# microsoft/ConfigNet

Hardware: AMD Instinct MI355X
Metric: train-step images/sec at 256x256 (G+D fwd+bwd) (higher is better)
Workload: dtype f32; 1 GPU; ConfigNet second-stage iteration (D + synth-D + latent-D + G + EMA), 256x256, batch 16 per GPU, fp32, Keras-Adam; global_batch=16, resolution=256, latent_dim=145, parallelism=dp1, losses_finite=True

## Files before the change

### confignet_amd/_lib.py

```python
import ctypes
import os

_HERE = os.path.dirname(os.path.abspath(__file__))
LIB_PATH = os.environ.get("CN_LIB") or os.path.join(_HERE, "libconfignet_hip.so")


class CnSumJob(ctypes.Structure):
    _fields_ = [("src", ctypes.c_void_p), ("dst", ctypes.c_void_p), ("count", ctypes.c_longlong), ("parts", ctypes.c_int),
                ("accumulate", ctypes.c_int)]


class CnDepthJob(ctypes.Structure):
    _fields_ = [("a", ctypes.c_void_p), ("b", ctypes.c_void_p), ("c", ctypes.c_void_p), ("m", ctypes.c_int), ("n", ctypes.c_int),
                ("k", ctypes.c_int), ("lda", ctypes.c_int), ("ldb", ctypes.c_int), ("ldc", ctypes.c_int)]


class CnRowsJob(ctypes.Structure):
    _fields_ = [("a", ctypes.c_void_p), ("b", ctypes.c_void_p), ("c", ctypes.c_void_p), ("bias", ctypes.c_void_p), ("mask", ctypes.c_void_p)] + \
               [(n_, ctypes.c_int) for n_ in ("m", "n", "k", "lda", "ldb", "ldc", "tb", "act", "accumulate")] + [("slope", ctypes.c_float)]


class CnGanJob(ctypes.Structure):
    _fields_ = [("s", ctypes.c_void_p), ("out", ctypes.c_void_p), ("gout", ctypes.c_void_p), ("n", ctypes.c_int), ("label", ctypes.c_float)]

# ... 40 lines not shown
    "cn_conv_wgrad_thin_partials": [],
    "cn_conv_wgrad_thin": [_G, _p, _p, _p, _p, _i, _p],
    "cn_conv_wgrad": [_G, _p, _p, _p, _i, _p],
    "cn_conv_wgrad_workspace_bytes": [_G],
    "cn_conv_wgrad_ws": [_G, _p, _p, _p, _i, _p, _z, _p],
    "cn_conv_wgrad_ws_slabs": [_G, _p, _p, _p, _i, _p, _z, ctypes.POINTER(_i), _p],
    "cn_conv_wgrad_dt_workspace_bytes": [_G, _i, _i, ctypes.POINTER(_z)],
    "cn_conv_wgrad_dt": [_G, _p, _i, _p, _i, _p, _i, _p, _z, ctypes.POINTER(_i), _p],
    "cn_conv_wgrad_plan": [_G, _i, _i, _i, ctypes.c_uint, _i, ctypes.POINTER(ctypes.c_longlong)],
    "cn_sum_parts_grouped": [_p, _i, _p],
    "cn_gemm_depth_grouped": [_p, _i, _p],
    "cn_gan_loss_grouped": [_p, _i, _i, _p],
    "cn_gemm_rows_grouped": [_p, _i, _p],
    "cn_conv_tune": [_i, _i, ctypes.c_long],
    "cn_conv_fwd_plan": [_G, _i, _i, _i, _i, _i, _i, _i, ctypes.POINTER(ctypes.c_int * 8)],
    "cn_conv_loop_select": [_i, _i, _i, _i],
    "cn_conv_fwd_dt": [_p, _p, _i, _p, _p, _p, _i, _i, _f, _p],
    "cn_conv_dgrad_dt": [_p, _p, _i, _p, _p, _i, _p],
    "cn_conv_wgrad_c3_partials": [],
    "cn_conv_wgrad_c3": [_p, _p, _p, _i, _p, _p, _i, _p],
    "cn_conv_wino_filter": [_p, _p, _i, _i, _i, _p],
    "cn_conv_fwd_wino": [_i, _i, _i, _i, _i, _p, _p, _p, _p, _i, _f, _p],
    "cn_conv_fwd_wino4": [_i, _i, _i, _i, _i, _p, _p, _p, _p, _i, _f, _p],
    "cn_conv_wino4_filter": [_p, _p, _i, _i, _i, _p],
    "cn_sumpool2": [_p, _p, _i, _i, _i, _i, _i, _i, _i, _p],
    "cn_gemm": [_i, _i, _i, _i, _i, _p, _i, _p, _i, _p, _i, _p, _i, _f, _p],
    "cn_gemm_plan": [_i] * 10 + [ctypes.POINTER(ctypes.c_int * 9)],
    "cn_nc_reduce4": [_p, _p, _i, _i, _i, _f, _i, _i, _p],
    "cn_nc_reduce": [_p, _p, _p, _p, _i, _i, _i, _i, _f, _i, _p],
    "cn_nc_reduce_plan": [_i, _i, _i, _i, _i, _i, ctypes.POINTER(ctypes.c_int * 8)],
    "cn_nc_lin2": [_p, _p, _p, _p, _p, _p, _p, _p, _i, _i, _i, _i, _i, _f, _i, _p],
    "cn_nc_rows_plan": [ctypes.c_longlong, _i, _i, ctypes.POINTER(ctypes.c_int * 2)],
    "cn_norm_coef_fwd": [_i, _p, _p, _p, _p, _p, _p, _p, _p, _i, _i, _i, _f, _p, _i, _p],
    "cn_norm_coef_bwd": [_i, _p, _p, _p, _p, _p, _p, _p, _p, _p, _p, _i, _i, _i, _f, _p],
    "cn_dual_tail_coef_fwd": [_p] * 13 + [_i, _i, _i, _f, _i, _i, _p],
    "cn_dual_tail_coef_bwd": [_p] * 13 + [ctypes.POINTER(ctypes.c_void_p), _i, _i, _i, _f, _i, _i, _p],
    "cn_dual_tail_gx": [_p] * 12 + [_i, _i, _i, _f, _i, _i, _p],
    "cn_dual_tail_gx_tx": [_p] * 18 + [_i, _i, _i, _f, _i, _i, _i, _p],
    "cn_norm_apply": [_i, _i] + [_p] * 13 + [_i, _i, _i, _f, _i, _f, _i, _p],
    "cn_nc_reduce_hxt": [_p, _p, _p, _p, _i, _i, _i, _f, _i, _i, _i, _p],
    "cn_zero": [_p, ctypes.c_size_t, _p],
    "cn_set_deterministic": [_i],
    "cn_get_deterministic": [],
    "cn_det_release_stream": [_p],
    "cn_gemm_acc": [_i, _i, _i, _i, _i, _p, _i, _p, _i, _p, _i, _p],
    "cn_sum_rows_into": [_p, _p, _i, _i, _i, _p],
# ... 61 lines not shown
```

### confignet_amd/csrc/common.h

```cpp
#pragma once
#include <hip/hip_runtime.h>
#include <stdint.h>
#include <stdio.h>
#include "../../include/confignet_hip.h"

void cn_set_error(const char* fmt, ...);

#define CN_CHECK_ARG(cond, ...)            \
    do {                                   \
        if (!(cond)) {                     \
            cn_set_error(__VA_ARGS__);     \
            return CN_EINVAL;              \
        }                                  \
    } while (0)

#define CN_HIP(expr)                                                              \
    do {                                                                          \
        hipError_t e__ = (expr);                                                  \
        if (e__ != hipSuccess) {                                                  \
            cn_set_error("%s failed: %s (%s:%d)", #expr, hipGetErrorString(e__), __FILE__, __LINE__); \
            return CN_EHIP;                                                       \
        }                                                                         \
    } while (0)

// ... 60 lines not shown

__device__ __forceinline__ void divmod_pos(int m, int d, int& q, int& r) {
    if ((d & (d - 1)) == 0) {
        q = m >> (__builtin_ctz(d));
        r = m & (d - 1);
    } else {
        q = m / d;
        r = m - q * d;
    }
}

__device__ __forceinline__ float cn_apply_act(float v, int act, float slope) {
    switch (act) {
        case CN_ACT_LRELU: return v > 0.f ? v : v * slope;
        case CN_ACT_RELU: return v > 0.f ? v : 0.f;
        case CN_ACT_TANH: return tanhf(v);
        default: break;
    }
    if (act == CN_ACT_RELU6) return fminf(fmaxf(v, 0.f), 6.f);
    if (act == CN_ACT_SIGMOID) return __fdividef(1.f, 1.f + __expf(-v));
    return v;
}

static inline int cn_cdiv(long a, long b) { return (int)((a + b - 1) / b); }

int cn_cu_count();
```

### confignet_amd/csrc/elementwise.hip

```cpp
#include "common.h"
#include "typed.h"
#include <stdlib.h>

namespace {

__device__ __forceinline__ float lrelu(float v, float s) { return v > 0.f ? v : v * s; }

__device__ __forceinline__ float act_deriv(float o, int act, float slope) {
    if (act == CN_ACT_LRELU) return o > 0.f ? 1.f : slope;
    if (act == CN_ACT_RELU) return o > 0.f ? 1.f : 0.f;
    if (act == CN_ACT_TANH) return 1.f - o * o;
    return 1.f;
}


template <int V> struct RowV { float v[V]; };

template <int V, typename T>
__device__ __forceinline__ RowV<V> ld_row(const T* p) {
    RowV<V> r;
    if constexpr (V == 4) {
        const float4 t = ld4<T>(p);
        r.v[0] = t.x; r.v[1] = t.y; r.v[2] = t.z; r.v[3] = t.w;
    } else {
        r.v[0] = ldf<T>(p);
    }
    return r;
}
template <int V, typename T>
__device__ __forceinline__ void st_row(T* p, const RowV<V>& r) {
    if constexpr (V == 4) st4<T>(p, make_float4(r.v[0], r.v[1], r.v[2], r.v[3]));
    else stf<T>(p, r.v[0]);
}

template <int Q, int V, typename Op>
__device__ __forceinline__ void nc_reduce_rows(Op op, float* const (&out)[Q], int S, int C, int rows_per_block, float* __restrict__ parts) {
// ... 616 lines not shown
    }
}

template <typename T>
__global__ void maxpool_fwd_kernel(const T* __restrict__ x, T* __restrict__ y, int n, int h, int w, int c,
                                   int oh, int ow, int k, int s, int pad) {
    const long total = (long)n * oh * ow * c;
    for (long i = (long)blockIdx.x * blockDim.x + threadIdx.x; i < total; i += (long)gridDim.x * blockDim.x) {
        const int ch = (int)(i % c);
        long t = i / c;
        const int ox = (int)(t % ow);
        t /= ow;
        const int oy = (int)(t % oh);
        const int b = (int)(t / oh);
        float best = -INFINITY;
        for (int dy = 0; dy < k; ++dy)
            for (int dx = 0; dx < k; ++dx) {
                const int iy = oy * s - pad + dy, ix = ox * s - pad + dx;
                const bool in = iy >= 0 && iy < h && ix >= 0 && ix < w;
                const float v = in ? ldf<T>(x + (((long)b * h + iy) * w + ix) * c + ch) : 0.f;
                if (in || pad > 0) best = fmaxf(best, v);
            }
        stf<T>(y + i, best);
    }
}

template <int V, typename T>
__global__ void avgpool3_same_kernel(const T* __restrict__ x, T* __restrict__ y, int n, int h, int w, int c) {
    const int CG = c / V;
    const long total = (long)n * h * w * CG;
    for (long i = (long)blockIdx.x * blockDim.x + threadIdx.x; i < total; i += (long)gridDim.x * blockDim.x) {
        const int cg = (int)(i % CG);
        long t = i / CG;
        const int ox = (int)(t % w);
        t /= w;
        const int oy = (int)(t % h);
        const int b = (int)(t / h);
        float acc[V];
#pragma unroll
        for (int e = 0; e < V; ++e) acc[e] = 0.f;
        int cnt = 0;
        for (int dy = -1; dy <= 1; ++dy)
            for (int dx = -1; dx <= 1; ++dx) {
                const int iy = oy + dy, ix = ox + dx;
                if (iy < 0 || iy >= h || ix < 0 || ix >= w) continue;
                const T* p = x + (((long)b * h + iy) * w + ix) * c + (long)cg * V;
// ... 552 lines not shown
    CN_LAUNCH_CHECK();
    return CN_OK;
}
extern "C" int cn_tap_bwd(const void* y, const void* target, const void* g, const float* s, void* out, int n, size_t row, float k,
                          int act, float slope, int dt, void* stream) {
    CN_CHECK_ARG(y && target && s && out && n > 0 && row > 0 && (dt == CN_F32 || dt == CN_BF16), "tap_bwd: bad args");
    const int vec = alv(y, dt) && alv(target, dt) && alv(out, dt) && (!g || alv(g, dt)) && row % 4 == 0;
    int bpr = (int)((row + 256 * 16 - 1) / (256 * 16));
    if (bpr > 512) bpr = 512;
    CN_DISPATCH_DT(dt, hipLaunchKernelGGL((tap_bwd_kernel<T>), dim3(bpr, n), dim3(256), 0, (hipStream_t)stream, (const T*)y, (const T*)target,
                                          (const T*)g, s, (T*)out, row, k, vec, act, slope));
    CN_LAUNCH_CHECK();
    return CN_OK;
}
extern "C" int cn_masked_diff(const float* a, const float* b, const uint8_t* mask, float* out, size_t pixels, int c, void* stream) {
    CN_CHECK_ARG(a && mask && out && c > 0, "masked_diff: bad args");
    if (!pixels) return CN_OK;
    EW_LAUNCH(masked_diff_kernel, pixels, a, b, mask, out, pixels, c)
}
extern "C" int cn_maxpool_fwd(const void* x, void* y, int n, int h, int w, int c, int k, int s, int pad, int dt, void* stream) {
    CN_CHECK_ARG(x && y && n > 0 && h > 0 && w > 0 && c > 0 && k > 0 && s > 0 && pad >= 0 && (dt == CN_F32 || dt == CN_BF16), "maxpool: bad args");
    const int oh = (h + 2 * pad - k) / s + 1, ow = (w + 2 * pad - k) / s + 1;
    const size_t total = (size_t)n * oh * ow * c;
    CN_DISPATCH_DT(dt, hipLaunchKernelGGL((maxpool_fwd_kernel<T>), dim3(ew_blocks(total)), dim3(256), 0, (hipStream_t)stream, (const T*)x, (T*)y, n, h, w, c, oh, ow, k, s, pad));
    CN_LAUNCH_CHECK();
    return CN_OK;
}
extern "C" int cn_avgpool3_same(const void* x, void* y, int n, int h, int w, int c, int dt, void* stream) {
    CN_CHECK_ARG(x && y && n > 0 && h > 0 && w > 0 && c > 0 && (dt == CN_F32 || dt == CN_BF16), "avgpool3_same: bad args");
    const bool v4 = c % 4 == 0 && alv(x, dt) && alv(y, dt);
    const size_t total = (size_t)n * h * w * (v4 ? c / 4 : c);
    CN_DISPATCH_DT(dt, {
        if (v4) hipLaunchKernelGGL((avgpool3_same_kernel<4, T>), dim3(ew_blocks(total)), dim3(256), 0, (hipStream_t)stream, (const T*)x, (T*)y, n, h, w, c);
        else hipLaunchKernelGGL((avgpool3_same_kernel<1, T>), dim3(ew_blocks(total)), dim3(256), 0, (hipStream_t)stream, (const T*)x, (T*)y, n, h, w, c);
    });
    CN_LAUNCH_CHECK();
    return CN_OK;
}
extern "C" int cn_maxpool_bwd(const void* x, const void* gy, void* gx, int n, int h, int w, int c, int k, int s, int pad, int dt, void* stream) {
    CN_CHECK_ARG(x && gy && gx && n > 0 && h > 0 && w > 0 && c > 0 && k > 0 && s > 0 && pad >= 0 && (dt == CN_F32 || dt == CN_BF16), "maxpool_bwd: bad args");
    const int oh = (h + 2 * pad - k) / s + 1, ow = (w + 2 * pad - k) / s + 1;
    const size_t total = (size_t)n * h * w * c;
    if (k == 2 && s == 2 && pad == 0 && h % 2 == 0 && w % 2 == 0 && c % 4 == 0 && alv(x, dt) && alv(gy, dt) && alv(gx, dt)) {
        const long windows4 = (long)n * oh * ow * (c / 4);
        CN_DISPATCH_DT(dt, hipLaunchKernelGGL((maxpool2_bwd_kernel<T>), dim3(ew_blocks((size_t)windows4)), dim3(256), 0, (hipStream_t)stream,
                                              (const T*)x, (const T*)gy, (T*)gx, windows4, oh, ow, c / 4));
// ... 206 lines not shown
```

### confignet_amd/csrc/winograd4.hip

```cpp
#include "common.h"

#include "mma_tile.h"

namespace {

typedef __attribute__((address_space(3))) float lds_float4;
typedef float v2f __attribute__((ext_vector_type(2)));

struct Wino4Geom {
    int n, h, w, cin, cout, bh, bw;
};

__global__ void wino4_filter_kernel(const float* __restrict__ W, float* __restrict__ U, int cin, int cout, int dgrad) {
    const long total = (long)cin * cout;
    for (long e = (long)blockIdx.x * blockDim.x + threadIdx.x; e < total; e += (long)gridDim.x * blockDim.x) {
        const int co = (int)(e % cout), ci = (int)(e / cout);
        float g[3][3];
#pragma unroll
        for (int a = 0; a < 3; ++a)
#pragma unroll
            for (int b = 0; b < 3; ++b)
                g[a][b] = dgrad ? W[((long)((2 - a) * 3 + (2 - b)) * cin + ci) * cout + co] : W[((long)(a * 3 + b) * cin + ci) * cout + co];
        float t[6][3];
#pragma unroll
// ... 17 lines not shown
            u[2] = (-1.f / 6.f) * (t0 - t1 + t2);
            u[3] = (1.f / 24.f) * t0 + (1.f / 12.f) * t1 + (1.f / 6.f) * t2;
            u[4] = (1.f / 24.f) * t0 - (1.f / 12.f) * t1 + (1.f / 6.f) * t2;
            u[5] = t2;
#pragma unroll
            for (int b = 0; b < 6; ++b) U[((long)(a * 6 + b) * kdim + k) * ndim + nn] = u[b];
        }
    }
}

#ifndef W4_ABLATE
#define W4_ABLATE 0
#endif
constexpr int W4_KC = 4;
constexpr int W4_T = 32;
constexpr int W4_C = 64;
constexpr int W4_VP = 40;
constexpr int W4_U = 36 * W4_KC * W4_C;
constexpr int W4_RAW_PIECES = 21;
constexpr int W4_RAW = W4_RAW_PIECES * 256;
constexpr int W4_BUF = 2 * W4_U + 2 * W4_RAW;


__global__ __launch_bounds__(768) void wino4_fwd_kernel(Wino4Geom g, const float* __restrict__ X, const float* __restrict__ U,
                                                        const float* __restrict__ bias, float* __restrict__ Y, int act, float slope) {
    __shared__ __attribute__((aligned(16))) float Vs[2][36][W4_KC][W4_VP];
    extern __shared__ __attribute__((aligned(16))) float BUF[];
    const int tid = threadIdx.x, lane = tid & 63, wave = __builtin_amdgcn_readfirstlane(tid >> 6);
    const int half = lane >> 5, l31 = lane & 31;
    const int wi = wave % 6, cb = wave / 6;

    const int nblk = g.n * g.bh * g.bw, total = nblk * (g.cout / W4_C);
    int wg = blockIdx.x;
    if (total % 8 == 0) wg = (wg & 7) * (total >> 3) + (wg >> 3);
    const int blk = wg % nblk, co0 = (wg / nblk) * W4_C;
    int img, brem, by, bx;
    divmod_pos(blk, g.bh * g.bw, img, brem);
    divmod_pos(brem, g.bw, by, bx);

    const __amdgpu_buffer_rsrc_t xres = __builtin_amdgcn_make_buffer_rsrc(const_cast<float*>(X), 0, g.n * g.h * g.w * g.cin * 4, 0x00020000);
    const __amdgpu_buffer_rsrc_t ures = __builtin_amdgcn_make_buffer_rsrc(const_cast<float*>(U), 0, 36 * g.cin * g.cout * 4, 0x00020000);

    unsigned uoff[3];
#pragma unroll
    for (int j = 0; j < 3; ++j) {
        const int p = wave + 12 * j;
        uoff[j] = (unsigned)((p * g.cin + (lane >> 4)) * g.cout + co0 + (lane & 15) * 4) * 4u;
    }
// ... 149 lines not shown
        float t = 0.f;
#pragma unroll
        for (int j = 0; j < 6; ++j)
#pragma unroll
            for (int r = 0; r < 16; ++r) t += acc[j][r];
        if (t == 12345.f) Y[tid] = t;
        return;
    }
    for (int rb = 0; rb < 2; ++rb) {
        if (cb == rb) {
#pragma unroll
            for (int e = 0; e < 16; ++e) {
                const int tl = 4 * half + (e & 3) + 8 * (e >> 2);
                const float a0 = acc[0][e], a1 = acc[1][e], a2 = acc[2][e], a3 = acc[3][e], a4 = acc[4][e], a5 = acc[5][e];
                const float s12 = a1 + a2, d12 = a1 - a2, s34 = a3 + a4, d34 = a3 - a4;
                float* dst = E + ((wi * 4) * 32 + tl) * 32 + l31;
                dst[0 * 1024] = a0 + s12 + s34;
                dst[1 * 1024] = d12 + 2.f * d34;
                dst[2 * 1024] = s12 + 4.f * s34;
                dst[3 * 1024] = d12 + 8.f * d34 + a5;
            }
        }
        __syncthreads();
        for (int idx = tid; idx < 1024; idx += 768) {
            const int c4 = idx & 7, tl = (idx >> 3) & 31, y = idx >> 8;
            float4 m[6];
#pragma unroll
            for (int i = 0; i < 6; ++i) m[i] = *reinterpret_cast<const float4*>(E + ((i * 4 + y) * 32 + tl) * 32 + 4 * c4);
            const int co = co0 + rb * 32 + 4 * c4;
            const float4 bv = bias ? *reinterpret_cast<const float4*>(bias + co) : make_float4(0.f, 0.f, 0.f, 0.f);
            const int otx = (tl & 3) + 4 * ((tl >> 3) & 1), oty = ((tl >> 2) & 1) + 2 * (tl >> 4);
            const int row0 = by * 16 + 4 * oty, col = bx * 32 + 4 * otx + y;
#define W4_O(f)                                                                                                          \
            const float s12##f = m[1].f + m[2].f, d12##f = m[1].f - m[2].f, s34##f = m[3].f + m[4].f, d34##f = m[3].f - m[4].f; \
            const float o0##f = m[0].f + s12##f + s34##f + bv.f, o1##f = d12##f + 2.f * d34##f + bv.f,                     \
                        o2##f = s12##f + 4.f * s34##f + bv.f, o3##f = d12##f + 8.f * d34##f + m[5].f + bv.f;
            W4_O(x) W4_O(y) W4_O(z) W4_O(w)
#undef W4_O
            float* dst = Y + ((long)(img * g.h + row0) * g.w + col) * g.cout + co;
            const long rs = (long)g.w * g.cout;
            *reinterpret_cast<float4*>(dst) = make_float4(cn_apply_act(o0x, act, slope), cn_apply_act(o0y, act, slope), cn_apply_act(o0z, act, slope), cn_apply_act(o0w, act, slope));
            *reinterpret_cast<float4*>(dst + rs) = make_float4(cn_apply_act(o1x, act, slope), cn_apply_act(o1y, act, slope), cn_apply_act(o1z, act, slope), cn_apply_act(o1w, act, slope));
            *reinterpret_cast<float4*>(dst + 2 * rs) = make_float4(cn_apply_act(o2x, act, slope), cn_apply_act(o2y, act, slope), cn_apply_act(o2z, act, slope), cn_apply_act(o2w, act, slope));
            *reinterpret_cast<float4*>(dst + 3 * rs) = make_float4(cn_apply_act(o3x, act, slope), cn_apply_act(o3y, act, slope), cn_apply_act(o3z, act, slope), cn_apply_act(o3w, act, slope));
        }
        __syncthreads();
    }
}

}

extern "C" int cn_conv_wino4_filter(const float* w, float* u, int cin, int cout, int dgrad, void* stream) {
    CN_CHECK_ARG(w && u && cin > 0 && cout > 0, "wino4_filter: bad args");
    const long total = (long)cin * cout;
    const int blocks = (int)((total + 255) / 256 > 4096 ? 4096 : (total + 255) / 256);
    hipLaunchKernelGGL(wino4_filter_kernel, dim3(blocks), dim3(256), 0, (hipStream_t)stream, w, u, cin, cout, dgrad);
    CN_LAUNCH_CHECK();
    return CN_OK;
}

extern "C" int cn_conv_fwd_wino4(int n, int h, int w, int cin, int cout, const float* x, const float* u, const float* bias,
                                 float* y, int act, float slope, void* stream) {
    CN_CHECK_ARG(x && u && y && n > 0 && h > 0 && w > 0, "conv_fwd_wino4: bad args");
    if (h % 16 || w % 32 || cin % 16 || cout % W4_C) return CN_EUNSUPPORTED;
    CN_CHECK_ARG((double)n * h * w * (cin > cout ? cin : cout) * 4.0 < 2147483647.0 && 144.0 * cin * cout < 2147483647.0,
                 "tensor exceeds 2^31 bytes (buffer descriptors, 32-bit offsets)");
    Wino4Geom g{n, h, w, cin, cout, h / 16, w / 32};
    const long nblk = (long)n * g.bh * g.bw;
    constexpr size_t lds = sizeof(float) * W4_BUF;
    static bool attr_set = false;
    if (!attr_set) {
        CN_HIP(hipFuncSetAttribute(reinterpret_cast<const void*>(wino4_fwd_kernel), hipFuncAttributeMaxDynamicSharedMemorySize, (int)lds));
        attr_set = true;
    }
    hipStream_t s = (hipStream_t)stream;
    cn_prof_begin(s, 2.0 * 36.0 * (double)nblk * W4_T * cin * cout, 4.0 * ((double)n * h * w * (cin + cout) + 36.0 * cin * cout), CN_FAM_WINO);
    hipLaunchKernelGGL(wino4_fwd_kernel, dim3((unsigned)(nblk * (cout / W4_C))), dim3(768), lds, s, g, x, u, bias, y, act, slope);
    cn_prof_end(s);
    CN_LAUNCH_CHECK();
    return CN_OK;
}
```

### confignet_amd/dnn_models/vgg.py

```python
import numpy as np
import torch

from .. import functional as F
from ..nn import Net, he_normal
from ..ops import ACT_RELU, ConvSpec

VGG19_CFG = [64, 64, "P", 128, 128, "P", 256, 256, 256, 256, "P", 512, 512]
VGG16_CFG = [64, 64, "P", 128, 128, "P", 256, 256, 256, "P", 512, 512]
VGG19_TAPS = (0, 1, 5, 9)
VGG16_TAPS = (0, 1, 5, 8)
C3 = ConvSpec((3, 3))


class VGGFeatures(Net):
    def __init__(self, cfg, taps, rng=None):
        super().__init__()
        rng = rng or np.random.default_rng(1234)
        self.cfg, self.taps = cfg, taps
        cin = 3
        for i, item in enumerate(c for c in cfg if c != "P"):
            self.add_weight("conv%d/kernel" % i, he_normal(rng, (3, 3, cin, item)), trainable=False)
            self.add_weight("conv%d/bias" % i, np.zeros(item, np.float32), trainable=False)
            cin = item
        self.finalize()

    def __call__(self, x_pre):
        feats, ci, x = [], 0, x_pre
        for item in self.cfg:
            if item == "P":
                x = F.maxpool(x, 2, 2)
            else:
                x = F.conv(x, self.weights[2 * ci], self.weights[2 * ci + 1], C3, ACT_RELU)
                if ci in self.taps:
                    feats.append(x)
                ci += 1
        return feats


class VGGLossFn(torch.autograd.Function):

    @staticmethod
    def forward(ctx, net, x, sizes, *targets):
        from .. import ops
        x = x.contiguous()
        ys, feats, ci, t = [], [], 0, x
        for item in net.cfg:
            if item == "P":
                t = ops.maxpool_fwd(t, 2, 2, 0)
            else:
                w, b = net.weights[2 * ci], net.weights[2 * ci + 1]
                t = ops.conv_fwd(t, w, b, C3.geom(tuple(t.shape), w.shape[-1]), ACT_RELU)
                ys.append(t)
                if ci in net.taps:
                    feats.append(t)
                ci += 1
        n = x.shape[0]
        groups = [n] if sizes is None else list(sizes)
        terms = []
        for a, b in zip(feats, targets):
            per = a.numel() // n
            n0, row = 0, []
            for sz in groups:
                row.append(ops.sqdiff_sum(a[n0:n0 + sz], b[n0:n0 + sz], 1.0 / (sz * per)))
                n0 += sz
            terms.append(torch.cat(row) if len(row) > 1 else row[0])
        total = torch.stack(terms).sum(0)
        ctx.net, ctx.sizes, ctx.x_shape = net, sizes, tuple(x.shape)
        ctx.save_for_backward(x, *ys, *targets)
        ctx.counts = (len(ys),)
        return total.reshape(()) if sizes is None else total

    @staticmethod
    def backward(ctx, g):
        from .. import ops
        if torch.is_grad_enabled():
            raise RuntimeError("VGGLossFn is first-order only")
        net, sizes = ctx.net, ctx.sizes
        saved = ctx.saved_tensors
        (ny,) = ctx.counts
        x, ys, targets = saved[0], saved[1:1 + ny], saved[1 + ny:]
        n = x.shape[0]
        g = g.reshape(-1).float()
        tap_of = {ci: k for k, ci in enumerate(net.taps)}
        gcur, ci, pooled = None, ny, None
        for item in reversed(net.cfg):
            if item == "P":
                pooled, gcur = gcur, None
                continue
            ci -= 1
            y = ys[ci]
            s_ = k = None
            if ci in tap_of:
                per = y.numel() // n
                if sizes is None:
                    s_, k = g.contiguous(), 2.0 / (n * per)
                else:
                    s_ = torch.cat([g[i:i + 1].expand(sz) * (1.0 / (sz * per)) for i, sz in enumerate(sizes)]).contiguous()
                    k = 2.0
            gu = None
            if pooled is not None:
                gu = ops.maxpool2_bwd_relu(y, pooled, targets[tap_of[ci]] if s_ is not None else None, s_, k if s_ is not None else 0.0)
                if gu is None:
                    gcur = ops.maxpool_bwd(y, pooled, 2, 2, 0)
                pooled = None
            if gu is not None:
                pass
            elif s_ is not None:
                gu = ops.tap_bwd(y, targets[tap_of[ci]], gcur, s_, k, ACT_RELU)
            elif gcur is None:
                continue
            else:
                gu = ops.act_bwd(gcur, y, ACT_RELU)
            w = net.weights[2 * ci]
            in_shape = conv_input_shape(net.cfg, ci, ctx.x_shape)
            gcur = ops.conv_dgrad(gu, w, C3.geom(in_shape, w.shape[-1]))
        return None, gcur, None, *([None] * len(targets))


def conv_input_shape(cfg, ci, x_shape):
    n, h, w, c = x_shape
    k = -1
    for item in cfg:
        if item == "P":
            h, w = h // 2, w // 2
        else:
            k += 1
            if k == ci:
                return (n, h, w, c)
            c = item
    raise IndexError(ci)
```

### confignet_amd/ops.py

```python
import contextlib
import ctypes
import math
import os
import threading

import torch

from ._lib import CN_BF16, CN_EUNSUPPORTED, CN_F32, CN_U8, CnConvGeom, CnDepthJob, CnGanJob, CnRowsJob, CnSumJob, check, lib

ACT_NONE, ACT_LRELU, ACT_RELU, ACT_TANH, ACT_RELU6, ACT_SIGMOID = 0, 1, 2, 3, 4, 5

ACT_DTYPE = torch.float32


def set_activation_dtype(dtype):
    global ACT_DTYPE
    if isinstance(dtype, str):
        dtype = {"f32": torch.float32, "fp32": torch.float32, "float32": torch.float32, "bf16": torch.bfloat16,
                 "bfloat16": torch.bfloat16}[dtype]
    assert dtype in (torch.float32, torch.bfloat16)
    ACT_DTYPE = dtype


def _stream():
# ... 336 lines not shown
        rc = lib.cn_conv_fwd_dt(ctypes.byref(g), _ptr(x), CN_F32, _fptr(w), _fptr(bias), _ptr(y), CN_BF16, act, slope, _stream())
        if rc == 0:
            return y
        if rc != CN_EUNSUPPORTED:
            check(rc, "cn_conv_fwd_dt")
    y = torch.empty(geom_out_shape(g), device=x.device, dtype=torch.float32)
    if req is not None and out_dtype == torch.float32 and g.cout % 4 == 0 and (req[0] == "act" or act == ACT_NONE):
        nk = 2 if req[0] == "act" else 4
        mark = _active_pool.cur if _active_pool is not None else None
        st = zero_pool_alloc((nk, g.n, g.cout), x.device)
        if st is not None:
            rc = lib.cn_conv_fwd_stats(ctypes.byref(g), _ptr(_c(x)), _fptr(w), _fptr(bias), _ptr(y), act, slope, _ptr(st), 1 if nk == 2 else 2,
                                       req[1], _stream())
            if rc == 0:
                _stats.ready = (y.data_ptr(), tuple(y.shape), req[0], tuple(st[k] for k in range(nk)))
                return y
            if rc != CN_EUNSUPPORTED:
                check(rc, "cn_conv_fwd_stats")
            _active_pool.cur = mark
    check(lib.cn_conv_fwd(ctypes.byref(g), _ptr(x), _fptr(w), _fptr(bias), _ptr(y), act, slope, _stream()), "cn_conv_fwd")
    return cast(y, out_dtype)


def conv_fwd_res(x, w, bias, res, g, act=ACT_NONE, slope=0.0):
    assert act in (ACT_NONE, ACT_RELU)
    if ACT_DTYPE == torch.float32 and x.dtype == torch.float32 and res.dtype == torch.float32 and not _wino_ok(g, g.cin, g.cout):
        x, res = _c(x), _c(res)
        y = torch.empty(geom_out_shape(g), device=x.device, dtype=torch.float32)
        rc = lib.cn_conv_fwd_res(ctypes.byref(g), _ptr(x), _fptr(w), _fptr(bias), _ptr(res), _ptr(y), act, slope, _stream())
        if rc == 0:
            return y
        if rc != CN_EUNSUPPORTED:
            check(rc, "cn_conv_fwd_res")
    y = conv_fwd(x, w, bias, g)
    return nc_lin2(tuple(y.shape), y, None, res, None, None, flags=8 if act == ACT_RELU else 0)


def scale_columns_segments(src, seg, a, total):
    dst = torch.empty(total, device=src.device, dtype=torch.float32)
    check(lib.cn_scale_columns_segments(_fptr(src), _ptr(dst), _ptr(seg), _fptr(_c(a)), seg.shape[0], total, _stream()),
          "cn_scale_columns_segments")
    return dst


def weight_tflip(w):
    w = _c(w)
# ... 979 lines not shown
```

### include/confignet_hip.h

```cpp
#ifndef CONFIGNET_HIP_H
#define CONFIGNET_HIP_H
#include <stddef.h>
#include <stdint.h>

#ifdef __cplusplus
extern "C" {
#endif

#define CN_OK 0
#define CN_EINVAL (-1)
#define CN_EHIP (-2)
#define CN_EUNSUPPORTED (-3)

#define CN_F32 0
#define CN_BF16 1
#define CN_U8 2

#define CN_ACT_NONE 0
#define CN_ACT_LRELU 1
#define CN_ACT_RELU 2
#define CN_ACT_TANH 3
#define CN_ACT_RELU6 4
#define CN_ACT_SIGMOID 5

// ... 61 lines not shown
int cn_gemm_rows_grouped(const CnRowsJob* jobs, int njobs, void* stream);
typedef struct CnGanJob {
    const float* s;
    float* out;
    const float* gout;
    int n;
    float label;
} CnGanJob;
int cn_gan_loss_grouped(const CnGanJob* jobs, int njobs, int backward, void* stream);
int cn_conv_fwd_dt(const CnConvGeom* g, const void* x, int x_dt, const float* w, const float* bias, void* y, int y_dt, int act,
                   float slope, void* stream);
int cn_conv_dgrad_dt(const CnConvGeom* g, const void* gy, int gy_dt, const float* w_tflip, void* gu, int gu_dt, void* stream);
int cn_conv_wgrad_c3_partials(void);
int cn_conv_wgrad_c3(const CnConvGeom* g, const float* x, const void* gy, int gy_dt, float* scratch, float* gw, int accumulate,
                     void* stream);
int cn_conv_wgrad_thin_partials(void);
int cn_conv_wgrad_thin(const CnConvGeom* g, const float* x, const float* gy, float* scratch, float* gw, int accumulate, void* stream);
int cn_conv_wino_filter(const float* w, float* u, int cin, int cout, int dgrad, void* stream);
int cn_conv_fwd_wino(int n, int h, int w, int cin, int cout, const float* x, const float* u, const float* bias, float* y,
                     int act, float slope, void* stream);
int cn_conv_wino4_filter(const float* w, float* u, int cin, int cout, int dgrad, void* stream);
int cn_conv_fwd_wino4(int n, int h, int w, int cin, int cout, const float* x, const float* u, const float* bias,
                      float* y, int act, float slope, void* stream);
int cn_conv_tune(int cfg, int splits, long wg_blocks);
int cn_conv_fwd_plan(const CnConvGeom* g, int bt, int has_bias, int act, int has_res, int stats_mode, int x_dt, int y_dt, int out[8]);
int cn_conv_loop_select(int loop, int kb, int ns, int np);
int cn_sumpool2(const void* gu, void* gx, int nd, int n, int d, int h, int w, int c, int dt, void* stream);

int cn_conv_weight_prep_bf16(const float* w, uint16_t* wf, uint16_t* wd, int taps, int cin, int cout, void* stream);
int cn_conv_fwd_bf16(const CnConvGeom* g, const uint16_t* x, const uint16_t* wf, const float* bias, uint16_t* y,
                     int act, float slope, void* stream);
int cn_conv_dgrad_bf16(const CnConvGeom* g, const uint16_t* gy, const uint16_t* wd, uint16_t* gu, void* stream);
int cn_conv_wgrad_bf16(const CnConvGeom* g, const uint16_t* x, const uint16_t* gy, float* gw, int accumulate, void* stream);
int cn_upfold_weights(const float* w, float* wf, float* wd, int nd, const int* k3, const int* pad_lo3, int cin, int cout,
                      int* k2_out3, int* pad2_out3, void* stream);
int cn_upfold_wgrad(const float* gw2, float* gw, int nd, const int* k3, const int* pad_lo3, int cin, int cout,
                    int accumulate, void* stream);
int cn_cast(const void* src, int src_dt, void* dst, int dst_dt, size_t numel, void* stream);

int cn_gemm(int trans_a, int trans_b, int m, int n, int k, const float* a, int lda,
            const float* b, int ldb, float* c, int ldc, const float* bias, int act, float slope,
            void* stream);
int cn_gemm_plan(int trans_a, int trans_b, int m, int n, int k, int ldc, int has_bias, int act, int accumulate, int deterministic,
                 int out[9]);

int cn_set_deterministic(int on);
// ... 110 lines not shown
```

Baseline: 423.0 images/sec.

## Fuse maxpool and ReLU-mask epilogues into Winograd-4 VGG conv kernels

Adds epilogue variants to the Winograd F(4,3) forward kernel. One writes the 2x2 max-pooled output directly, optionally skipping the full-resolution output when it is not a tap. Another applies the ReLU derivative mask, plus an optional perceptual-tap gradient term, to dgrad outputs. The VGG perceptual-loss forward and backward use these to avoid separate maxpool, act_bwd and tap_bwd passes over large activations. A vectorised float4 maxpool kernel is also added. The cost is more complex kernel templates and extra epilogue register pressure.

```diff
diff --git a/confignet_amd/_lib.py b/confignet_amd/_lib.py
--- a/confignet_amd/_lib.py
+++ b/confignet_amd/_lib.py
@@ -86,6 +86,7 @@
     "cn_conv_wino_filter": [_p, _p, _i, _i, _i, _p],
     "cn_conv_fwd_wino": [_i, _i, _i, _i, _i, _p, _p, _p, _p, _i, _f, _p],
     "cn_conv_fwd_wino4": [_i, _i, _i, _i, _i, _p, _p, _p, _p, _i, _f, _p],
+    "cn_conv_fwd_wino4_ep": [_i, _i, _i, _i, _i, _p, _p, _p, _p, _i, _f, _i, _p, _p, _p, _p, _i, _f, _p],
     "cn_conv_wino4_filter": [_p, _p, _i, _i, _i, _p],
     "cn_sumpool2": [_p, _p, _i, _i, _i, _i, _i, _i, _i, _p],
     "cn_gemm": [_i, _i, _i, _i, _i, _p, _i, _p, _i, _p, _i, _p, _i, _f, _p],
diff --git a/confignet_amd/csrc/common.h b/confignet_amd/csrc/common.h
--- a/confignet_amd/csrc/common.h
+++ b/confignet_amd/csrc/common.h
@@ -106,6 +106,13 @@
     return v;
 }
 
+__device__ __forceinline__ float act_deriv(float o, int act, float slope) {
+    if (act == CN_ACT_LRELU) return o > 0.f ? 1.f : slope;
+    if (act == CN_ACT_RELU) return o > 0.f ? 1.f : 0.f;
+    if (act == CN_ACT_TANH) return 1.f - o * o;
+    return 1.f;
+}
+
 static inline int cn_cdiv(long a, long b) { return (int)((a + b - 1) / b); }
 
 int cn_cu_count();
diff --git a/confignet_amd/csrc/elementwise.hip b/confignet_amd/csrc/elementwise.hip
--- a/confignet_amd/csrc/elementwise.hip
+++ b/confignet_amd/csrc/elementwise.hip
@@ -5,13 +5,6 @@
 namespace {
 
 __device__ __forceinline__ float lrelu(float v, float s) { return v > 0.f ? v : v * s; }
-
-__device__ __forceinline__ float act_deriv(float o, int act, float slope) {
-    if (act == CN_ACT_LRELU) return o > 0.f ? 1.f : slope;
-    if (act == CN_ACT_RELU) return o > 0.f ? 1.f : 0.f;
-    if (act == CN_ACT_TANH) return 1.f - o * o;
-    return 1.f;
-}
 
 
 template <int V> struct RowV { float v[V]; };
@@ -674,6 +667,31 @@
                 if (in || pad > 0) best = fmaxf(best, v);
             }
         stf<T>(y + i, best);
+    }
+}
+
+template <typename T>
+__global__ void maxpool_fwd4_kernel(const T* __restrict__ x, T* __restrict__ y, int n, int h, int w, int c4,
+                                    int oh, int ow, int k, int s, int pad) {
+    const int total = n * oh * ow * c4;
+    for (int i = blockIdx.x * blockDim.x + threadIdx.x; i < total; i += gridDim.x * blockDim.x) {
+        const int cg = i % c4;
+        int t = i / c4;
+        const int ox = t % ow;
+        t /= ow;
+        const int oy = t % oh;
+        const int b = t / oh;
+        float best[4] = {-INFINITY, -INFINITY, -INFINITY, -INFINITY};
+        for (int dy = 0; dy < k; ++dy)
+            for (int dx = 0; dx < k; ++dx) {
+                const int iy = oy * s - pad + dy, ix = ox * s - pad + dx;
+                const bool in = iy >= 0 && iy < h && ix >= 0 && ix < w;
+                if (!in && pad == 0) continue;
+                float4 v = make_float4(0.f, 0.f, 0.f, 0.f);
+                if (in) v = ld4<T>(x + ((long)(b * h + iy) * w + ix) * c4 * 4 + cg * 4);
+                best[0] = fmaxf(best[0], v.x); best[1] = fmaxf(best[1], v.y); best[2] = fmaxf(best[2], v.z); best[3] = fmaxf(best[3], v.w);
+            }
+        st4<T>(y + (long)i * 4, make_float4(best[0], best[1], best[2], best[3]));
     }
 }
 
@@ -1272,6 +1290,12 @@
     CN_CHECK_ARG(x && y && n > 0 && h > 0 && w > 0 && c > 0 && k > 0 && s > 0 && pad >= 0 && (dt == CN_F32 || dt == CN_BF16), "maxpool: bad args");
     const int oh = (h + 2 * pad - k) / s + 1, ow = (w + 2 * pad - k) / s + 1;
     const size_t total = (size_t)n * oh * ow * c;
+    if (c % 4 == 0 && alv(x, dt) && alv(y, dt) && total / 4 < (1UL << 30) && (size_t)n * h * w * c / 4 < (1UL << 30)) {
+        CN_DISPATCH_DT(dt, hipLaunchKernelGGL((maxpool_fwd4_kernel<T>), dim3(ew_blocks(total / 4)), dim3(256), 0, (hipStream_t)stream,
+                                              (const T*)x, (T*)y, n, h, w, c / 4, oh, ow, k, s, pad));
+        CN_LAUNCH_CHECK();
+        return CN_OK;
+    }
     CN_DISPATCH_DT(dt, hipLaunchKernelGGL((maxpool_fwd_kernel<T>), dim3(ew_blocks(total)), dim3(256), 0, (hipStream_t)stream, (const T*)x, (T*)y, n, h, w, c, oh, ow, k, s, pad));
     CN_LAUNCH_CHECK();
     return CN_OK;
diff --git a/confignet_amd/csrc/winograd4.hip b/confignet_amd/csrc/winograd4.hip
--- a/confignet_amd/csrc/winograd4.hip
+++ b/confignet_amd/csrc/winograd4.hip
@@ -63,8 +63,16 @@
 constexpr int W4_BUF = 2 * W4_U + 2 * W4_RAW;
 
 
+enum { W4_EP_NONE = 0, W4_EP_POOL = 1, W4_EP_POOL_ONLY = 2, W4_EP_MASK = 3 };
+template <int EP> struct Wino4Ep {};
+template <> struct Wino4Ep<W4_EP_POOL> { float* P; };
+template <> struct Wino4Ep<W4_EP_POOL_ONLY> { float* P; };
+template <> struct Wino4Ep<W4_EP_MASK> { const float* Ym; const float* T; const float* S; int s_rows; float k; };
+
+template <int EP>
 __global__ __launch_bounds__(768) void wino4_fwd_kernel(Wino4Geom g, const float* __restrict__ X, const float* __restrict__ U,
-                                                        const float* __restrict__ bias, float* __restrict__ Y, int act, float slope) {
+                                                        const float* __restrict__ bias, float* __restrict__ Y, int act, float slope,
+                                                        Wino4Ep<EP> ep) {
     __shared__ __attribute__((aligned(16))) float Vs[2][36][W4_KC][W4_VP];
     extern __shared__ __attribute__((aligned(16))) float BUF[];
     const int tid = threadIdx.x, lane = tid & 63, wave = __builtin_amdgcn_readfirstlane(tid >> 6);
@@ -260,6 +268,7 @@
             }
         }
         __syncthreads();
+        if constexpr (EP == W4_EP_NONE) {
         for (int idx = tid; idx < 1024; idx += 768) {
             const int c4 = idx & 7, tl = (idx >> 3) & 31, y = idx >> 8;
             float4 m[6];
@@ -282,6 +291,76 @@
             *reinterpret_cast<float4*>(dst + 2 * rs) = make_float4(cn_apply_act(o2x, act, slope), cn_apply_act(o2y, act, slope), cn_apply_act(o2z, act, slope), cn_apply_act(o2w, act, slope));
             *reinterpret_cast<float4*>(dst + 3 * rs) = make_float4(cn_apply_act(o3x, act, slope), cn_apply_act(o3y, act, slope), cn_apply_act(o3z, act, slope), cn_apply_act(o3w, act, slope));
         }
+        } else {
+        auto column = [&](int c4, int tl, int y, float4 (&o)[4]) {
+            float4 m[6];
+#pragma unroll
+            for (int i = 0; i < 6; ++i) m[i] = *reinterpret_cast<const float4*>(E + ((i * 4 + y) * 32 + tl) * 32 + 4 * c4);
+            const int co = co0 + rb * 32 + 4 * c4;
+            const float4 bv = bias ? *reinterpret_cast<const float4*>(bias + co) : make_float4(0.f, 0.f, 0.f, 0.f);
+#define W4_O(f)                                                                                                          \
+            const float s12##f = m[1].f + m[2].f, d12##f = m[1].f - m[2].f, s34##f = m[3].f + m[4].f, d34##f = m[3].f - m[4].f; \
+            const float o0##f = m[0].f + s12##f + s34##f + bv.f, o1##f = d12##f + 2.f * d34##f + bv.f,                     \
+                        o2##f = s12##f + 4.f * s34##f + bv.f, o3##f = d12##f + 8.f * d34##f + m[5].f + bv.f;
+            W4_O(x) W4_O(y) W4_O(z) W4_O(w)
+#undef W4_O
+            o[0] = make_float4(cn_apply_act(o0x, act, slope), cn_apply_act(o0y, act, slope), cn_apply_act(o0z, act, slope), cn_apply_act(o0w, act, slope));
+            o[1] = make_float4(cn_apply_act(o1x, act, slope), cn_apply_act(o1y, act, slope), cn_apply_act(o1z, act, slope), cn_apply_act(o1w, act, slope));
+            o[2] = make_float4(cn_apply_act(o2x, act, slope), cn_apply_act(o2y, act, slope), cn_apply_act(o2z, act, slope), cn_apply_act(o2w, act, slope));
+            o[3] = make_float4(cn_apply_act(o3x, act, slope), cn_apply_act(o3y, act, slope), cn_apply_act(o3z, act, slope), cn_apply_act(o3w, act, slope));
+        };
+        const long rs = (long)g.w * g.cout;
+        if constexpr (EP == W4_EP_POOL || EP == W4_EP_POOL_ONLY) {
+            if (tid < 512) {
+                const int c4 = tid & 7, tl = (tid >> 3) & 31, yp = tid >> 8;
+                const int co = co0 + rb * 32 + 4 * c4;
+                const int otx = (tl & 3) + 4 * ((tl >> 3) & 1), oty = ((tl >> 2) & 1) + 2 * (tl >> 4);
+                const int row0 = by * 16 + 4 * oty, col = bx * 32 + 4 * otx + 2 * yp;
+                float4 o[2][4];
+#pragma unroll
+                for (int q = 0; q < 2; ++q) {
+                    column(c4, tl, 2 * yp + q, o[q]);
+                    if constexpr (EP == W4_EP_POOL) {
+                        float* dst = Y + ((long)(img * g.h + row0) * g.w + col + q) * g.cout + co;
+#pragma unroll
+                        for (int r = 0; r < 4; ++r) *reinterpret_cast<float4*>(dst + r * rs) = o[q][r];
+                    }
+                }
+                const int ph = g.h >> 1, pw = g.w >> 1;
+                float* pdst = ep.P + ((long)(img * ph + (row0 >> 1)) * pw + (col >> 1)) * g.cout + co;
+#pragma unroll
+                for (int r = 0; r < 2; ++r) {
+#define W4_MAX(f) fmaxf(fmaxf(fmaxf(fmaxf(-INFINITY, o[0][2 * r].f), o[1][2 * r].f), o[0][2 * r + 1].f), o[1][2 * r + 1].f)
+                    *reinterpret_cast<float4*>(pdst + r * (long)pw * g.cout) = make_float4(W4_MAX(x), W4_MAX(y), W4_MAX(z), W4_MAX(w));
+#undef W4_MAX
+                }
+            }
+        } else {
+            for (int idx = tid; idx < 1024; idx += 768) {
+                const int c4 = idx & 7, tl = (idx >> 3) & 31, y = idx >> 8;
+                float4 o[4];
+                column(c4, tl, y, o);
+                const int co = co0 + rb * 32 + 4 * c4;
+                const int otx = (tl & 3) + 4 * ((tl >> 3) & 1), oty = ((tl >> 2) & 1) + 2 * (tl >> 4);
+                const int row0 = by * 16 + 4 * oty, col = bx * 32 + 4 * otx + y;
+                const long off = ((long)(img * g.h + row0) * g.w + col) * g.cout + co;
+                const float f = ep.T ? ep.S[ep.s_rows == 1 ? 0 : img] * ep.k : 0.f;
+#pragma unroll
+                for (int r = 0; r < 4; ++r) {
+                    const float4 u = *reinterpret_cast<const float4*>(ep.Ym + off + r * rs);
+                    float4 v = o[r];
+                    if (ep.T) {
+                        const float4 t = *reinterpret_cast<const float4*>(ep.T + off + r * rs);
+                        float4 d = make_float4((u.x - t.x) * f, (u.y - t.y) * f, (u.z - t.z) * f, (u.w - t.w) * f);
+                        d.x += v.x; d.y += v.y; d.z += v.z; d.w += v.w;
+                        v = d;
+                    }
+                    *reinterpret_cast<float4*>(Y + off + r * rs) = make_float4(v.x * act_deriv(u.x, CN_ACT_RELU, 0.f), v.y * act_deriv(u.y, CN_ACT_RELU, 0.f),
+                                                                               v.z * act_deriv(u.z, CN_ACT_RELU, 0.f), v.w * act_deriv(u.w, CN_ACT_RELU, 0.f));
+                }
+            }
+        }
+        }
         __syncthreads();
     }
 }
@@ -297,24 +376,58 @@
     return CN_OK;
 }
 
+template <int EP>
+static int wino4_launch(int n, int h, int w, int cin, int cout, const float* x, const float* u, const float* bias, float* y, int act,
+                        float slope, Wino4Ep<EP> ep, double bytes, hipStream_t s) {
+    Wino4Geom g{n, h, w, cin, cout, h / 16, w / 32};
+    const long nblk = (long)n * g.bh * g.bw;
+    constexpr size_t lds = sizeof(float) * W4_BUF;
+    static bool attr_set = false;
+    if (!attr_set) {
+        CN_HIP(hipFuncSetAttribute(reinterpret_cast<const void*>(wino4_fwd_kernel<EP>), hipFuncAttributeMaxDynamicSharedMemorySize, (int)lds));
+        attr_set = true;
+    }
+    cn_prof_begin(s, 2.0 * 36.0 * (double)nblk * W4_T * cin * cout, bytes, CN_FAM_WINO);
+    hipLaunchKernelGGL((wino4_fwd_kernel<EP>), dim3((unsigned)(nblk * (cout / W4_C))), dim3(768), lds, s, g, x, u, bias, y, act, slope, ep);
+    cn_prof_end(s);
+    CN_LAUNCH_CHECK();
+    return CN_OK;
+}
+
 extern "C" int cn_conv_fwd_wino4(int n, int h, int w, int cin, int cout, const float* x, const float* u, const float* bias,
                                  float* y, int act, float slope, void* stream) {
     CN_CHECK_ARG(x && u && y && n > 0 && h > 0 && w > 0, "conv_fwd_wino4: bad args");
     if (h % 16 || w % 32 || cin % 16 || cout % W4_C) return CN_EUNSUPPORTED;
     CN_CHECK_ARG((double)n * h * w * (cin > cout ? cin : cout) * 4.0 < 2147483647.0 && 144.0 * cin * cout < 2147483647.0,
                  "tensor exceeds 2^31 bytes (buffer descriptors, 32-bit offsets)");
-    Wino4Geom g{n, h, w, cin, cout, h / 16, w / 32};
-    const long nblk = (long)n * g.bh * g.bw;
-    constexpr size_t lds = sizeof(float) * W4_BUF;
-    static bool attr_set = false;
-    if (!attr_set) {
-        CN_HIP(hipFuncSetAttribute(reinterpret_cast<const void*>(wino4_fwd_kernel), hipFuncAttributeMaxDynamicSharedMemorySize, (int)lds));
-        attr_set = true;
-    }
-    hipStream_t s = (hipStream_t)stream;
-    cn_prof_begin(s, 2.0 * 36.0 * (double)nblk * W4_T * cin * cout, 4.0 * ((double)n * h * w * (cin + cout) + 36.0 * cin * cout), CN_FAM_WINO);
-    hipLaunchKernelGGL(wino4_fwd_kernel, dim3((unsigned)(nblk * (cout / W4_C))), dim3(768), lds, s, g, x, u, bias, y, act, slope);
-    cn_prof_end(s);
-    CN_LAUNCH_CHECK();
-    return CN_OK;
-}
+    return wino4_launch<W4_EP_NONE>(n, h, w, cin, cout, x, u, bias, y, act, slope, Wino4Ep<W4_EP_NONE>{},
+                                    4.0 * ((double)n * h * w * (cin + cout) + 36.0 * cin * cout), (hipStream_t)stream);
+}
+
+extern "C" int cn_conv_fwd_wino4_ep(int n, int h, int w, int cin, int cout, const float* x, const float* u, const float* bias, float* y,
+                                    int act, float slope, int mode, float* pooled, const float* ym, const float* target, const float* s,
+                                    int s_rows, float k, void* stream) {
+    CN_CHECK_ARG(x && u && n > 0 && h > 0 && w > 0, "conv_fwd_wino4_ep: bad args");
+    if (h % 16 || w % 32 || cin % 16 || cout % W4_C) return CN_EUNSUPPORTED;
+    if (mode != CN_W4_EP_POOL && mode != CN_W4_EP_POOL_ONLY && mode != CN_W4_EP_MASK) return CN_EUNSUPPORTED;
+    const auto al16 = [](const void* p) { return ((size_t)p & 15) == 0; };
+    if (mode == CN_W4_EP_MASK) {
+        CN_CHECK_ARG(y && ym && (!target || (s && (s_rows == 1 || s_rows == n))), "conv_fwd_wino4_ep: MASK needs y, ym and, with a target, 1 or n scales");
+        if (!al16(y) || !al16(ym) || !al16(target)) return CN_EUNSUPPORTED;
+    } else {
+        CN_CHECK_ARG(pooled && (y || mode == CN_W4_EP_POOL_ONLY), "conv_fwd_wino4_ep: POOL needs y and pooled");
+        if (!al16(pooled) || !al16(y)) return CN_EUNSUPPORTED;
+    }
+    CN_CHECK_ARG((double)n * h * w * (cin > cout ? cin : cout) * 4.0 < 2147483647.0 && 144.0 * cin * cout < 2147483647.0,
+                 "tensor exceeds 2^31 bytes (buffer descriptors, 32-bit offsets)");
+    const double px = (double)n * h * w, flt = 36.0 * cin * cout;
+    hipStream_t st = (hipStream_t)stream;
+    if (mode == CN_W4_EP_POOL)
+        return wino4_launch<W4_EP_POOL>(n, h, w, cin, cout, x, u, bias, y, act, slope, Wino4Ep<W4_EP_POOL>{pooled},
+                                        4.0 * (px * (cin + 1.25 * cout) + flt), st);
+    if (mode == CN_W4_EP_POOL_ONLY)
+        return wino4_launch<W4_EP_POOL_ONLY>(n, h, w, cin, cout, x, u, bias, y, act, slope, Wino4Ep<W4_EP_POOL_ONLY>{pooled},
+                                             4.0 * (px * (cin + 0.25 * cout) + flt), st);
+    return wino4_launch<W4_EP_MASK>(n, h, w, cin, cout, x, u, bias, y, act, slope, Wino4Ep<W4_EP_MASK>{ym, target, s, s_rows, k},
+                                    4.0 * (px * (cin + (target ? 3.0 : 2.0) * cout) + flt), st);
+}
diff --git a/confignet_amd/dnn_models/vgg.py b/confignet_amd/dnn_models/vgg.py
--- a/confignet_amd/dnn_models/vgg.py
+++ b/confignet_amd/dnn_models/vgg.py
@@ -10,6 +10,17 @@
 VGG19_TAPS = (0, 1, 5, 9)
 VGG16_TAPS = (0, 1, 5, 8)
 C3 = ConvSpec((3, 3))
+VGG_FUSED_EPILOGUES = True
+
+
+def _pool_follows(cfg):
+    out, ci = set(), 0
+    for i, item in enumerate(cfg):
+        if item != "P":
+            if i + 1 < len(cfg) and cfg[i + 1] == "P":
+                out.add(ci)
+            ci += 1
+    return out
 
 
 class VGGFeatures(Net):
@@ -25,12 +36,22 @@
         self.finalize()
 
     def __call__(self, x_pre):
+        from .. import ops
         feats, ci, x = [], 0, x_pre
-        for item in self.cfg:
+        fuse = VGG_FUSED_EPILOGUES and not torch.is_grad_enabled()
+        pooled = None
+        for i, item in enumerate(self.cfg):
             if item == "P":
-                x = F.maxpool(x, 2, 2)
+                x, pooled = (F.maxpool(x, 2, 2) if pooled is None else pooled), None
             else:
-                x = F.conv(x, self.weights[2 * ci], self.weights[2 * ci + 1], C3, ACT_RELU)
+                w, b = self.weights[2 * ci], self.weights[2 * ci + 1]
+                r = None
+                if fuse and i + 1 < len(self.cfg) and self.cfg[i + 1] == "P":
+                    r = ops.conv_fwd_pool(x.contiguous(), w, b, C3.geom(tuple(x.shape), w.shape[-1]), ACT_RELU, 0.0, keep_full=ci in self.taps)
+                if r is not None:
+                    x, pooled = r
+                else:
+                    x = F.conv(x, w, b, C3, ACT_RELU)
                 if ci in self.taps:
                     feats.append(x)
                 ci += 1
@@ -44,12 +65,20 @@
         from .. import ops
         x = x.contiguous()
         ys, feats, ci, t = [], [], 0, x
-        for item in net.cfg:
+        pooled = None
+        for i, item in enumerate(net.cfg):
             if item == "P":
-                t = ops.maxpool_fwd(t, 2, 2, 0)
+                t, pooled = (ops.maxpool_fwd(t, 2, 2, 0) if pooled is None else pooled), None
             else:
                 w, b = net.weights[2 * ci], net.weights[2 * ci + 1]
-                t = ops.conv_fwd(t, w, b, C3.geom(tuple(t.shape), w.shape[-1]), ACT_RELU)
+                geom = C3.geom(tuple(t.shape), w.shape[-1])
+                r = None
+                if VGG_FUSED_EPILOGUES and i + 1 < len(net.cfg) and net.cfg[i + 1] == "P":
+                    r = ops.conv_fwd_pool(t, w, b, geom, ACT_RELU)
+                if r is not None:
+                    t, pooled = r
+                else:
+                    t = ops.conv_fwd(t, w, b, geom, ACT_RELU)
                 ys.append(t)
                 if ci in net.taps:
                     feats.append(t)
@@ -82,38 +111,55 @@
         n = x.shape[0]
         g = g.reshape(-1).float()
         tap_of = {ci: k for k, ci in enumerate(net.taps)}
-        gcur, ci, pooled = None, ny, None
+        before_pool, last_tap = _pool_follows(net.cfg), max(net.taps)
+
+        def tap_scale(ci):
+            per = ys[ci].numel() // n
+            if sizes is None:
+                return g.contiguous(), 2.0 / (n * per)
+            return torch.cat([g[i:i + 1].expand(sz) * (1.0 / (sz * per)) for i, sz in enumerate(sizes)]).contiguous(), 2.0
+
+        gcur, ci, pooled, stepped = None, ny, None, False
         for item in reversed(net.cfg):
             if item == "P":
                 pooled, gcur = gcur, None
                 continue
             ci -= 1
             y = ys[ci]
-            s_ = k = None
-            if ci in tap_of:
-                per = y.numel() // n
-                if sizes is None:
-                    s_, k = g.contiguous(), 2.0 / (n * per)
+            if stepped:
+                gu, stepped = gcur, False
+            else:
+                s_ = k = None
+                if ci in tap_of:
+                    s_, k = tap_scale(ci)
+                gu = None
+                if pooled is not None:
+                    gu = ops.maxpool2_bwd_relu(y, pooled, targets[tap_of[ci]] if s_ is not None else None, s_, k if s_ is not None else 0.0)
+                    if gu is None:
+                        gcur = ops.maxpool_bwd(y, pooled, 2, 2, 0)
+                    pooled = None
+                if gu is not None:
+                    pass
+                elif s_ is not None:
+                    gu = ops.tap_bwd(y, targets[tap_of[ci]], gcur, s_, k, ACT_RELU)
+                elif gcur is None:
+                    continue
                 else:
-                    s_ = torch.cat([g[i:i + 1].expand(sz) * (1.0 / (sz * per)) for i, sz in enumerate(sizes)]).contiguous()
-                    k = 2.0
-            gu = None
-            if pooled is not None:
-                gu = ops.maxpool2_bwd_relu(y, pooled, targets[tap_of[ci]] if s_ is not None else None, s_, k if s_ is not None else 0.0)
-                if gu is None:
-                    gcur = ops.maxpool_bwd(y, pooled, 2, 2, 0)
-                pooled = None
-            if gu is not None:
-                pass
-            elif s_ is not None:
-                gu = ops.tap_bwd(y, targets[tap_of[ci]], gcur, s_, k, ACT_RELU)
-            elif gcur is None:
-                continue
-            else:
-                gu = ops.act_bwd(gcur, y, ACT_RELU)
+                    gu = ops.act_bwd(gcur, y, ACT_RELU)
             w = net.weights[2 * ci]
             in_shape = conv_input_shape(net.cfg, ci, ctx.x_shape)
-            gcur = ops.conv_dgrad(gu, w, C3.geom(in_shape, w.shape[-1]))
+            geom = C3.geom(in_shape, w.shape[-1])
+            gcur = None
+            if VGG_FUSED_EPILOGUES and ci >= 1 and ci - 1 not in before_pool and ci - 1 != last_tap:
+                yp = ys[ci - 1]
+                if ci - 1 in tap_of:
+                    sp, kp = tap_scale(ci - 1)
+                    gcur = ops.conv_dgrad_masked(gu, w, geom, yp, targets[tap_of[ci - 1]], sp, kp)
+                else:
+                    gcur = ops.conv_dgrad_masked(gu, w, geom, yp)
+                stepped = gcur is not None
+            if gcur is None:
+                gcur = ops.conv_dgrad(gu, w, geom)
         return None, gcur, None, *([None] * len(targets))
 
 
diff --git a/confignet_amd/ops.py b/confignet_amd/ops.py
--- a/confignet_amd/ops.py
+++ b/confignet_amd/ops.py
@@ -382,6 +382,37 @@
     return cast(y, out_dtype)
 
 
+W4_EP_POOL, W4_EP_POOL_ONLY, W4_EP_MASK = 1, 2, 3
+
+
+def conv_fwd_pool(x, w, bias, g, act=ACT_NONE, slope=0.0, keep_full=True):
+    if not (ACT_DTYPE == torch.float32 and x.dtype == torch.float32 and _wino4_ok(g, g.cin, g.cout)):
+        return None
+    _stats.request = _stats.ready = None
+    y = torch.empty(geom_out_shape(g), device=x.device, dtype=torch.float32) if keep_full else None
+    pooled = torch.empty((g.n, g.in_h // 2, g.in_w // 2, g.cout), device=x.device, dtype=torch.float32)
+    check(lib.cn_conv_fwd_wino4_ep(g.n, g.in_h, g.in_w, g.cin, g.cout, _ptr(_c(x)), _ptr(_wino4_filter(w, False)), _fptr(bias), _ptr(y),
+                                   act, slope, W4_EP_POOL if keep_full else W4_EP_POOL_ONLY, _ptr(pooled), None, None, None, 1, 0.0,
+                                   _stream()), "cn_conv_fwd_wino4_ep")
+    prof_note_saved(wino4_saved_flops(g))
+    return y, pooled
+
+
+def conv_dgrad_masked(gy, w, g, y, target=None, s=None, k=0.0):
+    if not (ACT_DTYPE == torch.float32 and gy.dtype == torch.float32 and y.dtype == torch.float32 and _wino4_ok(g, g.cout, g.cin)):
+        return None
+    if target is not None and (target.dtype != torch.float32 or s is None or s.numel() not in (1, g.n)):
+        return None
+    _log_mask(y, ACT_RELU)
+    gu = torch.empty(geom_in_shape(g, upsampled=True), device=gy.device, dtype=torch.float32)
+    check(lib.cn_conv_fwd_wino4_ep(g.n, g.in_h, g.in_w, g.cout, g.cin, _ptr(_c(gy)), _ptr(_wino4_filter(w, True)), None, _ptr(gu),
+                                   ACT_NONE, 0.0, W4_EP_MASK, None, _ptr(_c(y)), None if target is None else _ptr(_c(target)),
+                                   None if target is None else _fptr(s), 1 if target is None else s.numel(), k, _stream()),
+          "cn_conv_fwd_wino4_ep")
+    prof_note_saved(wino4_saved_flops(g))
+    return gu
+
+
 def conv_fwd_res(x, w, bias, res, g, act=ACT_NONE, slope=0.0):
     assert act in (ACT_NONE, ACT_RELU)
     if ACT_DTYPE == torch.float32 and x.dtype == torch.float32 and res.dtype == torch.float32 and not _wino_ok(g, g.cin, g.cout):
diff --git a/include/confignet_hip.h b/include/confignet_hip.h
--- a/include/confignet_hip.h
+++ b/include/confignet_hip.h
@@ -107,6 +107,12 @@
 int cn_conv_wino4_filter(const float* w, float* u, int cin, int cout, int dgrad, void* stream);
 int cn_conv_fwd_wino4(int n, int h, int w, int cin, int cout, const float* x, const float* u, const float* bias,
                       float* y, int act, float slope, void* stream);
+#define CN_W4_EP_POOL 1
+#define CN_W4_EP_POOL_ONLY 2
+#define CN_W4_EP_MASK 3
+int cn_conv_fwd_wino4_ep(int n, int h, int w, int cin, int cout, const float* x, const float* u, const float* bias, float* y,
+                         int act, float slope, int mode, float* pooled, const float* ym, const float* target, const float* s,
+                         int s_rows, float k, void* stream);
 int cn_conv_tune(int cfg, int splits, long wg_blocks);
 int cn_conv_fwd_plan(const CnConvGeom* g, int bt, int has_bias, int act, int has_res, int stats_mode, int x_dt, int y_dt, int out[8]);
 int cn_conv_loop_select(int loop, int kb, int ns, int np);
```

After: 427.4 images/sec (median of 6 runs). 1.01x the previous value.
